# LiHaoxu/SpMV-Research

Measured on AMD Instinct MI355X. Metric: GFLOP/s (2*nnz/t, fp64 SpMV y=A*x); achieved HBM GB/s and % of peak in 'roofline', higher is better.
Workload: dtype f64; 1 GPU; nlpkkt240 (synthetic twin); format=MI355X_SELLD_64_16384_d_v7, rows=27993600, cols=27993600, nnz=765374392, parallelism=single GPU

## Files before the change

spmv-research_amd/csrc/build_sell.hip:

```cpp
#include "handle.hpp"

namespace spmv {

static std::vector<int>
sigma_sort(const int * rp, long m, long sigma)
{
	std::vector<int> row_of_sorted(std::max<long>(m, 1));
	const long num_windows = (m + sigma - 1) / sigma;
	#pragma omp parallel for num_threads(spmv::host_threads()) schedule(dynamic, 4)
	for (long w = 0; w < num_windows; w++)
	{
		long s = w * sigma, e = std::min(m, s + sigma);
		int maxlen = 0;
		for (long i = s; i < e; i++)
			maxlen = std::max(maxlen, rp[i + 1] - rp[i]);
		std::vector<long> cnt((size_t) maxlen + 2, 0);
		for (long i = s; i < e; i++)
			cnt[maxlen - (rp[i + 1] - rp[i]) + 1]++;
		for (int b = 0; b <= maxlen; b++)
			cnt[b + 1] += cnt[b];
		for (long i = s; i < e; i++)
			row_of_sorted[s + cnt[maxlen - (rp[i + 1] - rp[i])]++] = (int) i;
	}
	return row_of_sorted;
// ... 64 lines not shown
					val[p] = va[js + k];
				}
				else
				{
					col[p] = pad_col;
					val[p] = 0.0;
				}
			}
		}
	}
	A->sell_slices = num_slices;
	A->sell_nnz_ext = nnz_ext;
	A->cfg.map = xcd_map_balanced(slice_ptr.data(), num_slices, slices_per_tile,
			resolve_remap(A->remap, (num_slices + slices_per_tile - 1) / slices_per_tile));
	if (dev_alloc(&A->d_slice_ptr, (size_t) num_slices + 1))
		return 1;
	HIP_TRY(hipMemcpy(A->d_slice_ptr, slice_ptr.data(), ((size_t) num_slices + 1) * sizeof(int64_t), hipMemcpyHostToDevice));
	if (upload_ints(col.data(), (size_t) nnz_ext, &A->d_col))
		return 1;
	if (upload_values(A, val.data(), (size_t) nnz_ext, &A->d_val))
		return 1;
	if (upload_ints(row_of_sorted.data(), (size_t) m, &A->d_row_of_sorted))
		return 1;
	A->mem_footprint = (double) (num_slices + 1) * sizeof(int64_t) + (double) nnz_ext * (A->vbytes + 4) + (double) m * 4;
	return 0;
}

static unsigned long long
sell5_exceptions(const int * rp, const int * ci, const int * rows, long maxlen, int r, bool & hard)
{
	unsigned long long mask = 0;
	hard = false;
	const int * cr = ci + rp[rows[r]];
	for (int l = 0; l < 64; l++)
	{
		const int * cl = ci + rp[rows[l]];
		const int off = cl[0] - cr[0];
		for (long k = 1; k < maxlen; k++)
		{
			const int d = cl[k] - cr[k] - off;
			if (d != 0)
				mask |= 1ull << l;
			if (d < -128 || d > 127)
				hard = true;
		}
	}
	return mask;
}

static void
sell_delta_map(spmv_mi355x_matrix * A, const int64_t * val_ptr)
{
	const long num_slices = A->sell_slices;
	const long spt = sell_slices_per_tile() / A->sell_split;
	A->cfg.map = xcd_map_balanced(val_ptr, num_slices, spt, resolve_remap(A->remap, (num_slices + spt - 1) / spt));
	A->mem_footprint = (double) (num_slices + 1) * 16 + (double) A->sell_val_words * A->vbytes + (double) A->sell_idx_bytes + (double) A->m * 4;
}

static void
sell_delta_install(spmv_mi355x_matrix * A, const SellDeltaArrays & r)
{
	A->d_row_of_sorted = r.row_of_sorted;
	A->d_sell_desc = r.desc;
	A->d_sell_idx = r.idx;
	A->d_val = r.val;
	std::copy(r.mode_counts, r.mode_counts + 4, A->sell_mode_slices);
	A->sell_v7_slices = r.v7_slices;
	A->sell_slices = (long) r.val_ptr.size() - 1;
	A->sell_nnz_ext = r.nnz_ext;
	A->sell_val_words = r.val_words;
	A->sell_idx_bytes = r.idx_bytes;
	sell_delta_map(A, r.val_ptr.data());
}

static void
sell_delta_names(spmv_mi355x_matrix * A, const spmv_mi355x_opts & o)
{
	const char * pf = A->f32 ? "f" : "d";
	const char * v7 = A->sell_v7_slices ? "_v7" : "";
	if (A->sell_split > 1)
		snprintf(A->format_name, sizeof(A->format_name), "MI355X_SELLD_%d_%ld_w%d_%s%s", A->sell_c, A->sell_sigma, A->sell_split, pf, v7);
	else
		snprintf(A->format_name, sizeof(A->format_name), "MI355X_SELLD_%d_%ld_%s%s", A->sell_c, A->sell_sigma, pf, v7);
	snprintf(A->kernel_name, sizeof(A->kernel_name), "sell_delta_kernel");
	if (A->sell_v7_slices && o.nontemporal == 0)
		A->cfg.nt = A->mem_footprint > 192.0 * 1024 * 1024 ? 1 : 0;
}

static int
build_sell_delta(spmv_mi355x_matrix * A, int sell_values, const int * rp, const int * ci, const double * va)
{
	const long m = A->m;
	constexpr int C = SELL_DELTA_C;
	const long sigma = A->sell_sigma;
	const long num_slices = (m + C - 1) / C;
	if (A->convert_on_device)
	{
		SellDeltaArrays r;
		if (sell_delta_convert_device(A->f32, m, A->n, A->nnz, sigma, sell_values, rp, ci, va, r))
			return 1;
		sell_delta_install(A, r);
		return 0;
	}
	const std::vector<int> row_of_sorted = sigma_sort(rp, m, sigma);
	std::vector<int64_t> val_ptr((size_t) num_slices + 1, 0), idx_ptr((size_t) num_slices + 1, 0);
	std::vector<unsigned char> mode((size_t) std::max<long>(num_slices, 1), 4);
	#pragma omp parallel for num_threads(spmv::host_threads()) schedule(dynamic, 64)
	for (long sl = 0; sl < num_slices; sl++)
	{
		long width = 0;
		const long i_e = std::min(m, (sl + 1) * C);
		for (long i = sl * C; i < i_e; i++)
		{
			int o = row_of_sorted[i];
			width = std::max<long>(width, rp[o + 1] - rp[o]);
		}
		const long maxlen = width;
		width = (width + 3) / 4 * 4;
		long maxdelta = 0;
		bool equal_len = (sl + 1) * C <= m && A->n >= C && maxlen > 0;
		for (long i = sl * C; i < i_e && equal_len; i++)
			equal_len = (rp[row_of_sorted[i] + 1] - rp[row_of_sorted[i]]) == maxlen;
		bool rowoff = equal_len;
		bool affine = (sl + 1) * C <= m && A->n >= C && maxlen == 0;
		if (rowoff)
		{
			const int o0 = row_of_sorted[sl * C];
			affine = true;
			for (long i = sl * C; i < i_e && rowoff; i++)
			{
				const int o = row_of_sorted[i];
				const int off = ci[rp[o]] - ci[rp[o0]];
				if (off != (int) (i - sl * C))
					affine = false;
				for (long k = 1; k < maxlen && rowoff; k++)
					rowoff = ci[rp[o] + k] - ci[rp[o0] + k] == off;
			}
			if (!rowoff)
				affine = false;
		}
		for (long k = 0; k < width; k++)
		{
			int lo = 0x7fffffff, hi = -1;
			for (long i = sl * C; i < i_e; i++)
			{
				int o = row_of_sorted[i];
				if (k < rp[o + 1] - rp[o])
				{
					int c = ci[rp[o] + k];
					lo = std::min(lo, c);
					hi = std::max(hi, c);
				}
			}
			if (hi >= 0)
				maxdelta = std::max<long>(maxdelta, (long) hi - lo);
		}
		int ref = -1, nex = 0;
		if (equal_len && !rowoff && !(sell_modes_off() & 4))
			for (int r = 0; r < 4 && ref < 0; r++)
			{
				bool hard;
				const int e = __builtin_popcountll(sell5_exceptions(rp, ci, row_of_sorted.data() + sl * C, maxlen, r, hard));
				if (sell5_accepts(e, hard))
				{
					ref = r;
					nex = e;
				}
// ... 474 lines not shown
```

spmv-research_amd/csrc/kernels_sell.hip:

```cpp

#include <type_traits>

#include "sell_delta_read.hpp"

namespace spmv {

constexpr int SELL_BLOCK = 256;
constexpr int SELL_WAVES = SELL_BLOCK / WAVE;

template <typename T, int C, bool NT>
__global__ __launch_bounds__(SELL_BLOCK) void
sell_kernel(const int64_t * __restrict__ slice_ptr, const int * __restrict__ col, const T * __restrict__ val,
		const int * __restrict__ row_of_sorted, const T * __restrict__ x, T * __restrict__ y,
		int m, int num_slices, int beta, XcdMap map)
{
	unsigned tile = xcd_tile(blockIdx.x, map);
	if (tile == NO_TILE)
		return;
	const int lane = threadIdx.x % WAVE;
	const int slice = tile * SELL_WAVES + threadIdx.x / WAVE;
	if (slice >= num_slices)
		return;
	const int64_t p_s = slice_ptr[slice];
	const int64_t p_e = slice_ptr[slice + 1];
// ... 493 lines not shown
}

template <typename T, int S, bool NT, bool V7>
__global__ __launch_bounds__(SELL_BLOCK) void
sell_delta_split_kernel(const int64_t * __restrict__ desc, const unsigned char * __restrict__ idx, const T * __restrict__ val,
		const int * __restrict__ row_of_sorted, const T * __restrict__ x, T * __restrict__ y,
		int m, int num_slices, int beta, XcdMap map)
{
	constexpr int SPB = SELL_WAVES / S;
	__shared__ T s_part[SELL_WAVES][WAVE];
	unsigned tile = xcd_tile(blockIdx.x, map);
	if (tile == NO_TILE)
		return;
	const int lane = threadIdx.x % WAVE;
	const int wave = threadIdx.x / WAVE;
	const int w = __builtin_amdgcn_readfirstlane(wave % S);
	const int slice = __builtin_amdgcn_readfirstlane((int) (tile * SPB + wave / S));
	T s = 0;
	if (slice < num_slices)
		s = sell_delta_one<T, NT, V7>(desc, slice, idx, val, lane, x, w, S);
	s_part[wave][lane] = s;
	__syncthreads();
	if (w == 0 && slice < num_slices)
	{
		T t = s_part[wave][lane];
		#pragma unroll
		for (int u = 1; u < S; u++)
			t += s_part[wave + u][lane];
		const long sorted_row = (long) slice * WAVE + lane;
		if (sorted_row < m)
		{
			T * yp = y + row_of_sorted[sorted_row];
			*yp = beta ? *yp + t : t;
		}
	}
}

template <typename T, bool V7>
static int
sell_delta_launch(int S, const int64_t * desc, const unsigned char * idx, const void * val, const int * row_of_sorted, const void * x, void * y,
		int m, int num_slices, const LaunchCfg & cfg, hipStream_t stream, long * grid_out)
{
	unsigned grid = xcd_grid(cfg.map);
	if (grid_out)
		*grid_out = grid;
	if (grid == 0)
		return 0;
	#define SELLD_LAUNCH(K) hipLaunchKernelGGL(K, dim3(grid), dim3(SELL_BLOCK), 0, stream, desc, idx, (const T *) val, \
			row_of_sorted, (const T *) x, (T *) y, m, num_slices, cfg.beta, cfg.map)
	if (S == 1)
	{
		if (cfg.nt) SELLD_LAUNCH((sell_delta_kernel<T, true, V7>));
		else        SELLD_LAUNCH((sell_delta_kernel<T, false, V7>));
	}
	else if (S == 2)
	{
		if (cfg.nt) SELLD_LAUNCH((sell_delta_split_kernel<T, 2, true, V7>));
		else        SELLD_LAUNCH((sell_delta_split_kernel<T, 2, false, V7>));
	}
	else if (S == 4)
	{
		if (cfg.nt) SELLD_LAUNCH((sell_delta_split_kernel<T, 4, true, V7>));
		else        SELLD_LAUNCH((sell_delta_split_kernel<T, 4, false, V7>));
	}
	else
	{
		set_error("sell_delta: waves per slice must be 1, 2 or 4 (got %d)", S);
		return 1;
	}
	#undef SELLD_LAUNCH
	HIP_TRY(hipGetLastError());
	return 0;
}

int
launch_sell_delta(bool f32, int waves_per_slice, bool v7, const int64_t * desc, const unsigned char * idx, const void * val, const int * row_of_sorted,
		const void * x, void * y, int m, int num_slices, const LaunchCfg & cfg, hipStream_t stream, long * grid_out)
{
	if (f32 && v7)
	{
		set_error("sell_delta: 7-byte values are fp64 only");
		return 1;
	}
	return f32 ? sell_delta_launch<float, false>(waves_per_slice, desc, idx, val, row_of_sorted, x, y, m, num_slices, cfg, stream, grid_out)
	     : v7  ? sell_delta_launch<double, true>(waves_per_slice, desc, idx, val, row_of_sorted, x, y, m, num_slices, cfg, stream, grid_out)
	           : sell_delta_launch<double, false>(waves_per_slice, desc, idx, val, row_of_sorted, x, y, m, num_slices, cfg, stream, grid_out);
}

template <typename T, int C>
static int
sell_launch_c(const int64_t * slice_ptr, const int * col, const void * val, const int * row_of_sorted, const void * x, void * y,
		int m, int num_slices, const LaunchCfg & cfg, hipStream_t stream, long * grid_out)
{
	unsigned grid = xcd_grid(cfg.map);
	if (grid_out)
		*grid_out = grid;
	if (grid == 0)
		return 0;
	if (cfg.nt)
		hipLaunchKernelGGL((sell_kernel<T, C, true>), dim3(grid), dim3(SELL_BLOCK), 0, stream, slice_ptr, col, (const T *) val,
				row_of_sorted, (const T *) x, (T *) y, m, num_slices, cfg.beta, cfg.map);
	else
		hipLaunchKernelGGL((sell_kernel<T, C, false>), dim3(grid), dim3(SELL_BLOCK), 0, stream, slice_ptr, col, (const T *) val,
				row_of_sorted, (const T *) x, (T *) y, m, num_slices, cfg.beta, cfg.map);
	HIP_TRY(hipGetLastError());
	return 0;
}

template <typename T>
static int
sell_dispatch(int C, const int64_t * slice_ptr, const int * col, const void * val, const int * row_of_sorted, const void * x, void * y,
		int m, int num_slices, const LaunchCfg & cfg, hipStream_t stream, long * grid_out)
{
	if (C == SELL_WIDE_C)
	{
		const unsigned grid = xcd_grid(cfg.map);
		if (grid_out)
			*grid_out = grid;
		if (grid == 0)
			return 0;
		if (cfg.nt)
			hipLaunchKernelGGL((sell_wide_kernel<T, true>), dim3(grid), dim3(SELL_WIDE_C), 0, stream, slice_ptr, col, (const T *) val, row_of_sorted,
					(const T *) x, (T *) y, m, num_slices, cfg.beta, cfg.map);
		else
			hipLaunchKernelGGL((sell_wide_kernel<T, false>), dim3(grid), dim3(SELL_WIDE_C), 0, stream, slice_ptr, col, (const T *) val, row_of_sorted,
					(const T *) x, (T *) y, m, num_slices, cfg.beta, cfg.map);
		HIP_TRY(hipGetLastError());
		return 0;
	}
	switch (C)
	{
		case 16: return sell_launch_c<T, 16>(slice_ptr, col, val, row_of_sorted, x, y, m, num_slices, cfg, stream, grid_out);
		case 32: return sell_launch_c<T, 32>(slice_ptr, col, val, row_of_sorted, x, y, m, num_slices, cfg, stream, grid_out);
		case 64: return sell_launch_c<T, 64>(slice_ptr, col, val, row_of_sorted, x, y, m, num_slices, cfg, stream, grid_out);
	}
	set_error("sell: C must be 16, 32, 64 or 256 (got %d)", C);
	return 1;
}

int
launch_sell(bool f32, int C, const int64_t * slice_ptr, const int * col, const void * val, const int * row_of_sorted,
		const void * x, void * y, int m, int num_slices, const LaunchCfg & cfg, hipStream_t stream, long * grid_out)
{
	return f32 ? sell_dispatch<float>(C, slice_ptr, col, val, row_of_sorted, x, y, m, num_slices, cfg, stream, grid_out)
	           : sell_dispatch<double>(C, slice_ptr, col, val, row_of_sorted, x, y, m, num_slices, cfg, stream, grid_out);
}

}
```

spmv-research_amd/csrc/launch.hpp:

```cpp
#pragma once

#include <vector>

#include "common.hpp"
#include "sell_delta_layout.hpp"

namespace spmv {

struct LaunchCfg {
	XcdMap map;
	int nt;
	int beta;
	int unit;
	double unit_value;
	int kahan;
};

inline long csr_scalar_rows_per_tile() { return 256; }
inline long csr_vector_rows_per_tile(int lanes_per_row, int rows_per_group = 1) { return 256L / lanes_per_row * rows_per_group; }
inline long csr_stream_rows_per_tile(int rows_per_wave) { return 4L * rows_per_wave; }
inline long sell_slices_per_tile() { return 4; }
inline long coo_waves_per_tile() { return 4; }

int launch_csr_scalar(bool f32, const int * row_ptr, const int * col, const void * val, const void * x, void * y,
		int m, const LaunchCfg & cfg, hipStream_t stream, long * grid_out);
int launch_csr_vector(bool f32, int lanes_per_row, int rows_per_group, const int * row_ptr, const int * col, const void * val,
		const void * x, void * y, int m, const LaunchCfg & cfg, hipStream_t stream, long * grid_out);

int csr_stream_cap();
int launch_csr_stream(bool f32, int rows_per_wave, const int * row_ptr, const int * col, const void * val, const void * x, void * y,
		int m, const LaunchCfg & cfg, hipStream_t stream, long * grid_out);

int csr_stream_t_cap(int rows_per_wave);
int launch_csr_stream_t(bool f32, int rows_per_wave, const int * row_ptr, const int * col, const void * val, const void * x, void * y,
		int m, const LaunchCfg & cfg, hipStream_t stream, long * grid_out);

int csr_stream_d_cap(int rows_per_wave);
long csr_stream_d_rows_per_tile(int rows_per_wave);
int launch_csr_stream_d(bool f32, int rows_per_wave, const int * row_ptr, const int * col, const void * val, const void * x, void * y,
		int m, const LaunchCfg & cfg, hipStream_t stream, long * grid_out);
constexpr int STREAM_SLACK = 512;

int csr_window_lds_budget();
int launch_csr_window(bool f32, int lanes_per_row, const int * row_ptr, const void * col, int col16, const void * val, const void * x, void * y,
		const int * blk_row, const int * blk_lo, const int * blk_w, int lds_bytes, const LaunchCfg & cfg, hipStream_t stream,
		long * grid_out);

int merge_tile_items(bool f32, int items_per_thread);
int launch_merge_search(const int * row_ptr, int m, int nnz, int tile_items, int num_tiles, int * coords ,
		hipStream_t stream);
int launch_merge(bool f32, int items_per_thread, const int * row_ptr, const int * col, const void * val, const void * x, void * y,
		int m, int nnz, int num_tiles, const int * coords, int * carry_row, void * carry_val,
		const LaunchCfg & cfg, hipStream_t stream, long * grid_out);

int launch_sell(bool f32, int C, const int64_t * slice_ptr, const int * col, const void * val, const int * row_of_sorted,
		const void * x, void * y, int m, int num_slices, const LaunchCfg & cfg, hipStream_t stream, long * grid_out);

int launch_sell_delta(bool f32, int waves_per_slice, bool v7, const int64_t * desc, const unsigned char * idx, const void * val, const int * row_of_sorted,
		const void * x, void * y, int m, int num_slices, const LaunchCfg & cfg, hipStream_t stream, long * grid_out);

int launch_sell_delta_spmm(bool f32, int waves_per_slice, bool v7, const int64_t * desc, const unsigned char * idx, const void * val,
		const int * row_of_sorted, int k, const void * X, long ldx, void * Y, long ldy, int m, int num_slices, const LaunchCfg & cfg,
		hipStream_t stream, long * grid_out);
int launch_spmm_column_gather(bool f32, const void * X, long ldx, void * x, long n, hipStream_t stream);
int launch_spmm_column_scatter(bool f32, const void * y, void * Y, long ldy, long m, int beta, hipStream_t stream);

int sell_window_lds_budget();
int launch_sell_window(bool f32, int waves_per_slice, int slices_per_group, const int * grp, const int64_t * sdesc, const unsigned short * idx,
		const void * val, const int * row_of_sorted, const void * x, void * y, int m, int lds_window_bytes, const LaunchCfg & cfg,
		hipStream_t stream, long * grid_out);

int launch_sell_window_sym(bool f32, int waves_per_slice, int slices_per_group, const int * grp, const int64_t * sdesc, const unsigned short * idx,
		const void * val, const int * row_of_sorted, const void * x, void * y, int m, int lds_window_bytes, const LaunchCfg & cfg,
		hipStream_t stream, long * grid_out);

inline int
sell_modes_off()
{
	const char * e = getenv("SPMV_MI355X_SELL_MODES_OFF");
	return e ? atoi(e) & 7 : 0;
}

inline int
sell_values_env(int opt)
{
	const char * e = getenv("SPMV_MI355X_SELL_VALUES");
	return e ? atoi(e) : opt;
}

__host__ __device__ inline long
sellw_val_pos(long k, long r, bool f32)
{
	return f32 ? (k / 4) * 256 + r * 4 + (k & 3) : (k / 2) * 128 + r * 2 + (k & 1);
}

struct SellDeltaArrays {
	int * row_of_sorted = nullptr;
	int64_t * desc = nullptr;
	unsigned char * idx = nullptr;
	void * val = nullptr;
	std::vector<int64_t> val_ptr;
	long mode_counts[4] = {0, 0, 0, 0};
	int64_t nnz_ext = 0;
	int64_t idx_bytes = 0;
	int64_t val_words = 0;
	long v7_slices = 0;
};

int sell_delta_convert_device(bool f32, long m, long n_cols, long nnz, long sigma, int sell_values, const int * rp_host, const int * ci_host,
		const double * va_host, SellDeltaArrays & out);

int sell_delta_convert_resident(bool f32, long m, long n_cols, long nnz, long sigma, int sell_values, const int * rp, const int * ci,
		const double * va, SellDeltaArrays & out);
int blocked_entries_convert_device(bool f32, bool uniform, long m, long nnz, const int * rp_host, const int * ci_host, const double * va_host, long NR, int WGS, long CH,
		const std::vector<int> & range_row, const std::vector<int> & range_long, const std::vector<int> & long_row, const std::vector<int> & chunk_ptr,
		const std::vector<int> & chunk_row, const std::vector<int> & wg_rows, long SPAN, long BATCH, int slot_bits, int SPARE, long ghost_batches,
		std::vector<int> & batch_ptr, unsigned ** d_ent_out, void ** d_val_out, int ** d_batch_base_out);
int sell_plain_convert_device(bool f32, long m, long nnz, int C, int TPR, long sigma, const int * rp_host, const int * ci_host, const double * va_host,
		int64_t ** d_slice_ptr_out, int ** d_col_out, void ** d_val_out, int ** d_row_of_sorted_out, std::vector<int64_t> & slice_ptr_host);
int sell_window_convert_device(bool f32, long m, long nnz, int NS, bool sym, long lds_budget_bytes, const int * rp_host, const int * ci_host,
		const double * va_host, int ** d_grp_out, int ** d_row_of_sorted_out, int64_t ** d_desc_out, unsigned short ** d_idx_out, void ** d_val_out,
		std::vector<int64_t> & desc_host, int * max_w_out);

int coo_wave_items(int items_per_lane);
int launch_coo(bool f32, int items_per_lane, const int * rowind, const int * col, const void * val, const void * x, void * y,
		int m, long nnz, int num_waves, int * carry_row, void * carry_val,
		const LaunchCfg & cfg, hipStream_t stream, long * grid_out);

int coo_blocked_rows_cap(bool f32);
int coo_blocked_wgs_per_range();
int coo_blocked_chunk_rows();
int coo_blocked_batch_entries(bool unit);
int coo_blocked_spare_slots();
int coo_blocked_slot_bits();
int coo_blocked_max_long_rows();
int launch_coo_blocked(bool f32, const int * wg_rows, const int * range_row, const int * chunk_ptr, const int * chunk_row, const int * batch_ptr, const int * batch_base,
		const int * range_long,
		const int * long_row, int num_long, const unsigned * ent, const void * val, const void * x, void * y, void * carry, int num_ranges,
		int chunk_rows, int lds_bytes, const LaunchCfg & cfg, hipStream_t stream, long * grid_out);

int launch_expand_rows(const int * row_ptr, int m, int * rowind, hipStream_t stream);

}
```

spmv-research_amd/csrc/sell_delta_read.hpp:

```cpp
#pragma once

#include "launch.hpp"

namespace spmv {

typedef int sell_int4 __attribute__((ext_vector_type(4)));
typedef unsigned sell_uint2 __attribute__((ext_vector_type(2)));

template <typename T, bool NT>
__device__ __forceinline__ void
sell_group_values(const T * __restrict__ vp, T (&v)[4])
{
	typedef T T2 __attribute__((ext_vector_type(2)));
	const T2 w0 = ld_stream<NT>(reinterpret_cast<const T2 *>(vp));
	const T2 w1 = ld_stream<NT>(reinterpret_cast<const T2 *>(vp + 2 * WAVE));
	v[0] = w0.x;
	v[1] = w0.y;
	v[2] = w1.x;
	v[3] = w1.y;
}

template <typename T, bool NT, int NSTEPS>
__device__ __forceinline__ void
sell_tail_values(const T * __restrict__ vp, int lane, T (&v)[3])
{
	typedef T T2 __attribute__((ext_vector_type(2)));
	v[1] = v[2] = T(0);
	if (NSTEPS == 1)
		v[0] = ld_stream<NT>(vp - lane);
	else
	{
		const T2 w0 = ld_stream<NT>(reinterpret_cast<const T2 *>(vp));
		v[0] = w0.x;
		v[1] = w0.y;
		if (NSTEPS == 3)
			v[2] = ld_stream<NT>(vp + 2 * WAVE - lane);
	}
}

typedef unsigned sell_uint4 __attribute__((ext_vector_type(4)));
typedef unsigned sell_uint3 __attribute__((ext_vector_type(3), aligned(4)));

__device__ __forceinline__ double
sell_v7_value(unsigned h, unsigned k, unsigned lo)
{
	return __builtin_bit_cast(double, (unsigned long long) sell_v7_decode_hi(h, k) << 32 | lo);
}

template <typename T, bool NT, bool V7>
struct SellVals {
	const T * vp;
	int lane;
	unsigned k;
	__device__ __forceinline__ void group(int g, T (&v)[4]) const
	{
		if constexpr (!V7)
			sell_group_values<T, NT>(vp + (size_t) g * 4 * WAVE, v);
		else
		{
			static_assert(sizeof(T) == 8, "7-byte values are fp64 only");
			const unsigned char * b = reinterpret_cast<const unsigned char *>(vp) + (size_t) g * (8 * SELL_V7_GROUP_WORDS);
			const sell_uint4 lo = ld_stream<NT>(reinterpret_cast<const sell_uint4 *>(b));
			const sell_uint3 * hp = reinterpret_cast<const sell_uint3 *>(b + 1024 - 4 * lane);
			sell_uint3 hi;
			if constexpr (NT)
				hi = __builtin_nontemporal_load(hp);
			else
				hi = *hp;
			v[0] = sell_v7_value(hi.x, k, lo.x);
			v[1] = sell_v7_value(__builtin_amdgcn_alignbit(hi.y, hi.x, 24), k, lo.y);
			v[2] = sell_v7_value(__builtin_amdgcn_alignbit(hi.z, hi.y, 16), k, lo.z);
			v[3] = sell_v7_value(hi.z >> 8, k, lo.w);
		}
	}
	__device__ __forceinline__ const T * tail(int g) const { return vp + (size_t) g * (V7 ? SELL_V7_GROUP_WORDS : 4 * WAVE); }
};

template <int MODE>
struct SellDeltaIdx {
	sell_int4 base;
	sell_uint2 d;
};

template <int MODE, bool NT>
__device__ __forceinline__ void
sell_delta_load_idx(SellDeltaIdx<MODE> & q, const unsigned char * __restrict__ gp , int lane)
{
	q.base = *reinterpret_cast<const sell_int4 *>(gp);
	if constexpr (MODE == 1)
		q.d.x = ld_stream<NT>(reinterpret_cast<const unsigned *>(gp + 16) + lane);
	else
		q.d = ld_stream<NT>(reinterpret_cast<const sell_uint2 *>(gp + 16) + lane);
}

template <int MODE>
__device__ __forceinline__ void
sell_delta_cols(const SellDeltaIdx<MODE> & q, int (&c)[4])
{
	if constexpr (MODE == 1)
	{
		c[0] = q.base.x + (int) (q.d.x & 255u);
		c[1] = q.base.y + (int) ((q.d.x >> 8) & 255u);
		c[2] = q.base.z + (int) ((q.d.x >> 16) & 255u);
		c[3] = q.base.w + (int) (q.d.x >> 24);
	}
	else
	{
		c[0] = q.base.x + (int) (q.d.x & 0xffffu);
		c[1] = q.base.y + (int) (q.d.x >> 16);
		c[2] = q.base.z + (int) (q.d.y & 0xffffu);
		c[3] = q.base.w + (int) (q.d.y >> 16);
	}
}

struct SellDeltaIdx5 {
	sell_int4 base;
	unsigned d;
	sell_int4 corr;
};

template <bool NT, bool SCALAR>
__device__ __forceinline__ void
sell_delta_load_idx5(SellDeltaIdx5 & q, const unsigned char * __restrict__ gp , int rank)
{
	q.base = *reinterpret_cast<const sell_int4 *>(gp);
	if constexpr (SCALAR)
		q.corr = *reinterpret_cast<const sell_int4 *>(gp + 16);
	else
		q.d = ld_stream<NT>(reinterpret_cast<const unsigned *>(gp + 16) + rank);
}

template <bool SCALAR>
__device__ __forceinline__ void
sell_delta_cols5(const SellDeltaIdx5 & q, bool ex, int lane, int off, const int (&xl)[4], int (&c)[4])
{
	int d;
	if constexpr (SCALAR)
	{
		d = lane == xl[0] ? q.corr.x : 0;
		d = lane == xl[1] ? q.corr.y : d;
		d = lane == xl[2] ? q.corr.z : d;
		d = lane == xl[3] ? q.corr.w : d;
	}
	else
		d = ex ? (int) q.d : 0;
	c[0] = q.base.x + off + ((d << 24) >> 24);
	c[1] = q.base.y + off + ((d << 16) >> 24);
	c[2] = q.base.z + off + ((d << 8) >> 24);
	c[3] = q.base.w + off + (d >> 24);
}

template <int MODE, bool NT>
__device__ __forceinline__ void
sell_group_cols(const unsigned char * __restrict__ gp , int lane, int off, int (&c)[4])
{
	static_assert(MODE >= 0 && MODE <= 4, "mode 5 has its own reader (sell_delta_load_idx5, sell_delta_cols5)");
	if constexpr (MODE == 0 || MODE == 3)
	{
		const sell_int4 base = *reinterpret_cast<const sell_int4 *>(gp);
		c[0] = base.x + off;
// ... 46 lines not shown
```

spmv-research_amd/csrc/spmv_mi355x.hip:

```cpp

#include "handle.hpp"

namespace spmv {

static thread_local char g_err[1024] = "";

void
set_error(const char * fmt, ...)
{
	va_list ap;
	va_start(ap, fmt);
	vsnprintf(g_err, sizeof(g_err), fmt, ap);
	va_end(ap);
}

void
init_handle(spmv_mi355x_matrix * A, int format, int precision, int device, const spmv_mi355x_opts & o, long m, long n, long nnz)
{
	A->format = format;
	A->precision = precision;
	A->f32 = (precision == SPMV_MI355X_F32);
	A->vbytes = A->f32 ? 4 : 8;
	A->device = device;
	A->placement_level = (o.placement == 1 || o.placement == 3 || o.placement == 4) ? o.placement : 0;
// ... 462 lines not shown
		HIP_TRY(hipStreamCreate(&A->stream));
	if (!A->d_y && tune_placement(A))
		return 1;
	return 0;
}

void * spmv_mi355x_x_device(spmv_mi355x_matrix * A) { return ensure_xy(A) ? nullptr : A->d_x; }
void * spmv_mi355x_y_device(spmv_mi355x_matrix * A) { return ensure_xy(A) ? nullptr : A->d_y; }

int
spmv_mi355x_set_always_copy(spmv_mi355x_matrix * A, int on)
{
	A->always_copy = on != 0;
	return 0;
}

int
spmv_mi355x_upload_x(spmv_mi355x_matrix * A, const void * x_host)
{
	if (ensure_xy(A))
		return 1;
	HIP_TRY(hipDeviceSynchronize());
	HIP_TRY(hipMemcpyAsync(A->d_x, x_host, (size_t) A->n * A->vbytes, hipMemcpyHostToDevice, A->stream));
	HIP_TRY(hipStreamSynchronize(A->stream));
	A->cached_x_host = x_host;
	return 0;
}

int
spmv_mi355x_upload_y(spmv_mi355x_matrix * A, const void * y_host)
{
	if (ensure_xy(A))
		return 1;
	HIP_TRY(hipDeviceSynchronize());
	HIP_TRY(hipMemcpyAsync(A->d_y, y_host, (size_t) A->m * A->vbytes, hipMemcpyHostToDevice, A->stream));
	HIP_TRY(hipStreamSynchronize(A->stream));
	return 0;
}

int
spmv_mi355x_download_y(spmv_mi355x_matrix * A, void * y_host)
{
	if (ensure_xy(A))
		return 1;
	HIP_TRY(hipDeviceSynchronize());
	HIP_TRY(hipMemcpyAsync(y_host, A->d_y, (size_t) A->m * A->vbytes, hipMemcpyDeviceToHost, A->stream));
	HIP_TRY(hipStreamSynchronize(A->stream));
	A->y_downloaded = true;
	return 0;
}

int
spmv_mi355x_spmv(spmv_mi355x_matrix * A, const void * x_host, void * y_host)
{
	if (ensure_xy(A))
		return 1;
	if (A->always_copy || A->cached_x_host != x_host)
	{
		if (spmv_mi355x_upload_x(A, x_host))
			return 1;
		A->y_downloaded = false;
	}
	if (spmv_mi355x_spmv_device_async(A, A->d_x, A->d_y, 0, A->stream))
		return 1;
	HIP_TRY(hipStreamSynchronize(A->stream));
	if (A->always_copy || !A->y_downloaded)
		if (spmv_mi355x_download_y(A, y_host))
			return 1;
	return 0;
}

int
spmv_mi355x_stored_array(const spmv_mi355x_matrix * A, const char * name, void ** out, size_t * bytes_out)
{
	if (!A || !name || !out || !bytes_out)
	{
		set_error("stored_array: NULL argument");
		return 1;
	}
	*out = nullptr;
	*bytes_out = 0;
	struct Arr { const char * name; const void * p; size_t bytes; };
	std::vector<Arr> arrs;
	if (A->format == SPMV_MI355X_SELL_C_SIGMA && A->sell_window)
		arrs = {{"val", A->d_val, (size_t) A->sell_nnz_ext * A->vbytes}, {"idx", A->d_sell_idx, (size_t) A->sell_idx_bytes},
		        {"desc", A->d_sell_desc, 2 * ((size_t) A->sell_slices + 1) * 8}, {"row_of_sorted", A->d_row_of_sorted, (size_t) A->m * 4},
		        {"groups", A->d_sellw_grp, (size_t) A->sellw_groups * 16}};
	else if (A->format == SPMV_MI355X_SELL_C_SIGMA && A->sell_delta)
		arrs = {{"val", A->d_val, (size_t) A->sell_val_words * A->vbytes}, {"idx", A->d_sell_idx, (size_t) A->sell_idx_bytes},
		        {"desc", A->d_sell_desc, 2 * ((size_t) A->sell_slices + 1) * 8}, {"row_of_sorted", A->d_row_of_sorted, (size_t) A->m * 4}};
	else if (A->format == SPMV_MI355X_SELL_C_SIGMA)
		arrs = {{"val", A->d_val, (size_t) A->sell_nnz_ext * A->vbytes}, {"col", A->d_col, (size_t) A->sell_nnz_ext * 4},
		        {"slice_ptr", A->d_slice_ptr, ((size_t) A->sell_slices + 1) * 8}, {"row_of_sorted", A->d_row_of_sorted, (size_t) A->m * 4}};
	else if (A->d_coob_ent)
	{
		const size_t NT = (size_t) A->coob_ranges * spmv::coo_blocked_wgs_per_range(), BATCH = (size_t) spmv::coo_blocked_batch_entries(A->cfg.unit != 0);
		const size_t stored = ((size_t) A->coob_batches + 2) * BATCH;
		arrs = {{"entries", A->d_coob_ent, stored * 4}, {"val", A->d_val, A->cfg.unit ? 0 : stored * A->vbytes},
		        {"batch_base", A->d_coob_batch_base, stored / 64 * 4}, {"batch_ptr", A->d_coob_batch_ptr, (NT + 1) * 4},
		        {"chunk_ptr", A->d_coob_chunk_ptr, (NT + 1) * 4}, {"chunk_row", A->d_coob_chunk_row, (size_t) A->coob_chunks * 4},
		        {"wg_rows", A->d_coob_wg_rows, NT * 4}, {"range_row", A->d_coob_range_row, ((size_t) A->coob_ranges + 1) * 4},
		        {"range_long", A->d_coob_range_long, ((size_t) A->coob_ranges + 1) * 4}, {"long_row", A->d_coob_long_row, (size_t) A->coob_num_long * 4}};
	}
	else
	{
		set_error("stored_array: only for the SELL layouts and the column-blocked layout (this handle: %s)", A->format_name);
		return 1;
	}
	for (const Arr & a : arrs)
		if (!strcmp(a.name, name))
		{
			HIP_TRY(hipSetDevice(A->device));
			void * host = malloc(std::max<size_t>(a.bytes, 1));
			if (!host)
			{
				set_error("stored_array: out of host memory (%zu bytes)", a.bytes);
				return 1;
			}
			if (a.bytes && hipMemcpy(host, a.p, a.bytes, hipMemcpyDeviceToHost) != hipSuccess)
			{
				free(host);
				set_error("stored_array: copy failed: %s", hipGetErrorString(hipGetLastError()));
				return 1;
			}
			*out = host;
			*bytes_out = a.bytes;
			return 0;
		}
	set_error("stored_array: %s has no array '%s'", A->format_name, name);
	return 1;
}

int
spmv_mi355x_sell_layout(const spmv_mi355x_matrix * A, long * C_out, long * sigma_out, long * num_slices_out,
		long * nnz_ext_out, int64_t ** slice_ptr_out, int32_t ** col_out, double ** val_out, int32_t ** row_of_sorted_out)
{
	if (A->format != SPMV_MI355X_SELL_C_SIGMA)
	{
		set_error("not a SELL handle");
		return 1;
	}
	if (A->sell_window)
	{
		set_error("sell_layout: not available for the LDS-window layout (16-bit window-relative indices)");
		return 1;
	}
	HIP_TRY(hipSetDevice(A->device));
	if (C_out) *C_out = A->sell_c;
	if (sigma_out) *sigma_out = A->sell_sigma;
	if (num_slices_out) *num_slices_out = A->sell_slices;
	if (nnz_ext_out) *nnz_ext_out = A->sell_nnz_ext;
	std::vector<int64_t> h_desc, plain_ptr;
	std::vector<unsigned char> h_idx;
	if (A->sell_delta)
	{
		h_desc.resize(2 * ((size_t) A->sell_slices + 1));
		HIP_TRY(hipMemcpy(h_desc.data(), A->d_sell_desc, h_desc.size() * sizeof(int64_t), hipMemcpyDeviceToHost));
		h_idx.resize((size_t) std::max<long>(A->sell_idx_bytes, 1));
		HIP_TRY(hipMemcpy(h_idx.data(), A->d_sell_idx, (size_t) A->sell_idx_bytes, hipMemcpyDeviceToHost));
		plain_ptr.assign((size_t) A->sell_slices + 1, 0);
		for (long sl = 0; sl < A->sell_slices; sl++)
		{
			const long width = spmv::sell_slice_width(h_desc[2 * sl + 2] - h_desc[2 * sl], spmv::sell_desc_v7(h_desc[2 * sl + 1]));
			plain_ptr[sl + 1] = plain_ptr[sl] + width * 64;
		}
	}
// ... 134 lines not shown
```

Measured before the change: 1415 GFLOP/s.

## Add producer-wave LDS ring kernel for SELL-delta fp64 SpMV

Adds a new SELL-delta kernel in which a dedicated producer wave streams slice values into a double-buffered LDS ring with global_load_lds DMA, while four consumer waves gather x and run FMAs on values read from LDS. It is enabled automatically for fp64 single-wave slices when the extended value array exceeds 256 MiB, with a persistent grid capped per XCD. The aim is to overlap value streaming with x gathers and keep more bytes in flight toward HBM bandwidth. In exchange it adds block-wide barriers per round, imbalance when the four slices in a tile differ in length, and fewer resident workgroups.

```diff
diff --git a/spmv-research_amd/csrc/build_sell.hip b/spmv-research_amd/csrc/build_sell.hip
--- a/spmv-research_amd/csrc/build_sell.hip
+++ b/spmv-research_amd/csrc/build_sell.hip
@@ -170,7 +170,10 @@
 		snprintf(A->format_name, sizeof(A->format_name), "MI355X_SELLD_%d_%ld_w%d_%s%s", A->sell_c, A->sell_sigma, A->sell_split, pf, v7);
 	else
 		snprintf(A->format_name, sizeof(A->format_name), "MI355X_SELLD_%d_%ld_%s%s", A->sell_c, A->sell_sigma, pf, v7);
-	snprintf(A->kernel_name, sizeof(A->kernel_name), "sell_delta_kernel");
+	A->cfg.ring = sell_ring_wanted(A->f32, A->sell_split, A->sell_nnz_ext) ? 1 : 0;
+	snprintf(A->kernel_name, sizeof(A->kernel_name), A->cfg.ring ? "sell_delta_ring_kernel" : "sell_delta_kernel");
+	if (A->cfg.ring)
+		A->kernel_block = 320;
 	if (A->sell_v7_slices && o.nontemporal == 0)
 		A->cfg.nt = A->mem_footprint > 192.0 * 1024 * 1024 ? 1 : 0;
 }
diff --git a/spmv-research_amd/csrc/kernels_sell.hip b/spmv-research_amd/csrc/kernels_sell.hip
--- a/spmv-research_amd/csrc/kernels_sell.hip
+++ b/spmv-research_amd/csrc/kernels_sell.hip
@@ -599,6 +599,9 @@
 		set_error("sell_delta: 7-byte values are fp64 only");
 		return 1;
 	}
+	if (cfg.ring && !f32 && waves_per_slice == 1)
+		return launch_sell_delta_ring(v7, desc, idx, (const double *) val, row_of_sorted, (const double *) x, (double *) y, m, num_slices, cfg, stream,
+				grid_out);
 	return f32 ? sell_delta_launch<float, false>(waves_per_slice, desc, idx, val, row_of_sorted, x, y, m, num_slices, cfg, stream, grid_out)
 	     : v7  ? sell_delta_launch<double, true>(waves_per_slice, desc, idx, val, row_of_sorted, x, y, m, num_slices, cfg, stream, grid_out)
 	           : sell_delta_launch<double, false>(waves_per_slice, desc, idx, val, row_of_sorted, x, y, m, num_slices, cfg, stream, grid_out);
diff --git a/spmv-research_amd/csrc/kernels_sell_ring.hip b/spmv-research_amd/csrc/kernels_sell_ring.hip
--- /dev/null
+++ b/spmv-research_amd/csrc/kernels_sell_ring.hip
@@ -0,0 +1,339 @@
+
+#include "sell_delta_read.hpp"
+
+namespace spmv {
+
+constexpr int RING_NC = 4;
+constexpr int RING_D = 2;
+constexpr int RING_BLOCK = (RING_NC + 1) * WAVE;
+constexpr int RING_WG_PER_XCD = 32 * 2;
+constexpr int RING_LDS_BYTES = RING_NC * RING_D * SELL_RING_SLOT_BYTES;
+static_assert(RING_LDS_BYTES <= 65536, "the LDS-DMA destination base must stay below 64 KiB");
+
+struct RingSlice {
+	int64_t v_off, i_word;
+	int width, full;
+	bool v7;
+};
+
+template <bool V7>
+__device__ __forceinline__ RingSlice
+ring_slice_info(const int64_t * __restrict__ desc, int slice, int num_slices)
+{
+	RingSlice r{0, 0, 0, 0, false};
+	if (slice < num_slices)
+	{
+		r.v_off = desc[2 * slice];
+		r.i_word = desc[2 * slice + 1];
+		r.v7 = V7 && sell_desc_v7(r.i_word);
+		r.width = (int) sell_slice_width(desc[2 * slice + 2] - r.v_off, r.v7);
+		r.full = r.width / 4;
+	}
+	return r;
+}
+
+__device__ __forceinline__ int ring_trips(int full) { return (full + SELL_RING_SLOT_GROUPS - 1) / SELL_RING_SLOT_GROUPS; }
+
+template <bool V7>
+__device__ __forceinline__ int
+ring_tile_rounds(const int64_t * __restrict__ desc, unsigned tile, int num_slices)
+{
+	int R = 0;
+	#pragma unroll
+	for (int c = 0; c < RING_NC; c++)
+	{
+		const int t = ring_trips(ring_slice_info<V7>(desc, (int) (tile * RING_NC + c), num_slices).full);
+		R = t > R ? t : R;
+	}
+	return R;
+}
+
+template <typename F>
+__device__ __forceinline__ void
+ring_walk(const XcdMap & map, unsigned blocks, F && f)
+{
+	for (unsigned vb = blockIdx.x; vb < blocks; vb += gridDim.x)
+	{
+		const unsigned tile = xcd_tile(vb, map);
+		if (tile != NO_TILE)
+			f(tile);
+	}
+}
+
+__device__ __forceinline__ void
+ring_barrier()
+{
+	asm volatile("s_waitcnt lgkmcnt(0)" ::: "memory");
+	__builtin_amdgcn_s_barrier();
+	asm volatile("" ::: "memory");
+}
+
+__device__ __forceinline__ void
+ring_pin(double & v)
+{
+	asm volatile("" : "+v"(v));
+}
+
+template <int MODE, bool NT, bool V7, bool SC5>
+__device__ __forceinline__ double
+ring_slice(const RingSlice & si, const unsigned char * __restrict__ ip, int off, unsigned long long mask, const double * __restrict__ val,
+		const void * safe, int lane, const double * __restrict__ x, const unsigned char * slots, int & rnd)
+{
+	typedef double double2_t __attribute__((ext_vector_type(2)));
+	const int full = si.full, rem = si.width - 4 * full, trips = ring_trips(full), groups = (si.width + 3) / 4;
+	const Sell5Lane<SC5> l5(mask, lane);
+	const size_t GB = MODE == 5 ? sell_group_bytes(5, (unsigned) __popcll(mask)) : sell_group_bytes(MODE);
+	auto cols = [&](int g, int (&c)[4]) {
+		const unsigned char * gp = ip + (size_t) g * GB;
+		if constexpr (MODE == 5)
+		{
+			SellDeltaIdx5 q;
+			sell_delta_load_idx5<NT, SC5>(q, gp, l5.rank);
+			sell_delta_cols5<SC5>(q, l5.ex, lane, off, l5.xl, c);
+		}
+		else
+			sell_group_cols<MODE, NT>(gp, lane, off, c);
+	};
+	const double * tp = val + si.v_off + (size_t) full * (si.v7 ? SELL_V7_GROUP_WORDS : 4 * WAVE);
+	const double2_t * pa = rem >= 2 ? reinterpret_cast<const double2_t *>(tp + 2 * lane) : reinterpret_cast<const double2_t *>(safe);
+	const double * pb = rem == 1 ? tp + lane : rem == 3 ? tp + 2 * WAVE + lane : reinterpret_cast<const double *>(safe);
+	const double2_t ta = ld_stream<NT>(pa);
+	const double tb = ld_stream<NT>(pb);
+	const double tv0 = rem == 1 ? tb : ta.x, tv1 = ta.y, tv2 = tb;
+	int ct[4];
+	cols(groups - 1, ct);
+	const double tx0 = x[ct[0]], tx1 = x[ct[1]], tx2 = x[ct[2]];
+
+	const SellRingVals<V7> rv{lane, V7 ? (unsigned) (sell_v7_e0(si.i_word) - 1) << 20 : 0u};
+	double s = 0;
+	auto gather = [&](int q, double (&xx)[4][4]) {
+		#pragma unroll
+		for (int u = 0; u < 4; u++)
+		{
+			int g = 4 * q + u;
+			g = g < full ? g : full - 1;
+			int c[4];
+			cols(g, c);
+			#pragma unroll
+			for (int t = 0; t < 4; t++)
+				xx[u][t] = x[c[t]];
+		}
+	};
+	auto consume = [&](int q, const double (&xx)[4][4]) {
+		ring_barrier();
+		const unsigned char * slot = slots + (rnd % RING_D) * SELL_RING_SLOT_BYTES;
+		rnd++;
+		double v[4][4];
+		#pragma unroll
+		for (int u = 0; u < 4; u++)
+			rv.group(slot, u, v[u]);
+		#pragma unroll
+		for (int u = 0; u < 4; u++)
+			if (4 * q + u < full)
+			{
+				#pragma unroll
+				for (int t = 0; t < 4; t++)
+					s = fma(v[u][t], xx[u][t], s);
+			}
+	};
+	if (trips > 0)
+	{
+		double xa[4][4];
+		gather(0, xa);
+		for (int q = 0; q + 1 < trips; q++)
+		{
+			double xb[4][4];
+			gather(q + 1, xb);
+			consume(q, xa);
+			#pragma unroll
+			for (int u = 0; u < 4; u++)
+				#pragma unroll
+				for (int t = 0; t < 4; t++)
+				{
+					ring_pin(xb[u][t]);
+					xa[u][t] = xb[u][t];
+				}
+		}
+		consume(trips - 1, xa);
+	}
+	if (rem > 0) s = fma(tv0, tx0, s);
+	if (rem > 1) s = fma(tv1, tx1, s);
+	if (rem > 2) s = fma(tv2, tx2, s);
+	return s;
+}
+
+template <bool NT, bool V7, bool SV7>
+__device__ __forceinline__ double
+ring_slice_modes(const RingSlice & si, const unsigned char * __restrict__ idx, const double * __restrict__ val, const void * safe, int lane,
+		const double * __restrict__ x, const unsigned char * slots, int & rnd)
+{
+	const unsigned char * ip = idx + sell_desc_idx(si.i_word);
+	const int mode = sell_desc_mode(si.i_word);
+	if (mode == 0)
+		return ring_slice<0, NT, SV7, false>(si, ip, lane, 0ull, val, safe, lane, x, slots, rnd);
+	if (mode == 1)
+		return ring_slice<1, NT, SV7, false>(si, ip, lane, 0ull, val, safe, lane, x, slots, rnd);
+	if (mode == 2)
+		return ring_slice<2, NT, SV7, false>(si, ip, lane, 0ull, val, safe, lane, x, slots, rnd);
+	if (mode == 4)
+		return ring_slice<4, NT, SV7, false>(si, ip, lane, 0ull, val, safe, lane, x, slots, rnd);
+	const int off = ld_stream<NT>(reinterpret_cast<const int *>(ip) + lane);
+	if (mode == 3)
+		return ring_slice<3, NT, SV7, false>(si, ip + sell_header_bytes(3), off, 0ull, val, safe, lane, x, slots, rnd);
+	const unsigned long long mask = *reinterpret_cast<const unsigned long long *>(ip + 4 * WAVE);
+	if (__popcll(mask) <= 4)
+		return ring_slice<5, NT, SV7, true>(si, ip + sell_header_bytes(5), off, mask, val, safe, lane, x, slots, rnd);
+	return ring_slice<5, NT, SV7, false>(si, ip + sell_header_bytes(5), off, mask, val, safe, lane, x, slots, rnd);
+}
+
+typedef __attribute__((address_space(1))) const void ring_gvoid;
+typedef __attribute__((address_space(3))) void ring_lvoid;
+
+template <typename T, bool NT, bool V7>
+__global__ __launch_bounds__(RING_BLOCK) void
+sell_delta_ring_kernel(const int64_t * __restrict__ desc, const unsigned char * __restrict__ idx, const T * __restrict__ val,
+		const int * __restrict__ row_of_sorted, const T * __restrict__ x, T * __restrict__ y,
+		int m, int num_slices, int beta, XcdMap map, unsigned blocks)
+{
+	static_assert(sizeof(T) == 8, "the ring kernel is fp64 only");
+	__shared__ __attribute__((aligned(16))) unsigned char ring[RING_LDS_BYTES];
+	const int lane = threadIdx.x % WAVE;
+	const int wave = __builtin_amdgcn_readfirstlane((int) (threadIdx.x / WAVE));
+	int rnd = 0;
+	if (wave == RING_NC)
+	{
+		ring_walk(map, blocks, [&](unsigned tile) {
+			RingSlice si[RING_NC];
+			int R = 0;
+			#pragma unroll
+			for (int c = 0; c < RING_NC; c++)
+			{
+				si[c] = ring_slice_info<V7>(desc, (int) (tile * RING_NC + c), num_slices);
+				const int t = ring_trips(si[c].full);
+				R = t > R ? t : R;
+			}
+			for (int q = 0; q < R; q++)
+			{
+				unsigned char * base = ring + (rnd % RING_D) * SELL_RING_SLOT_BYTES;
+				#pragma unroll
+				for (int c = 0; c < RING_NC; c++)
+				{
+					const int n = si[c].full - SELL_RING_SLOT_GROUPS * q;
+					const size_t gb = si[c].v7 ? 8 * SELL_V7_GROUP_WORDS : SELL_RING_GROUP_BYTES;
+					const unsigned char * src = reinterpret_cast<const unsigned char *>(val + si[c].v_off) + (size_t) SELL_RING_SLOT_GROUPS * q * gb;
+					unsigned char * dst = base + c * RING_D * SELL_RING_SLOT_BYTES;
+					#pragma unroll
+					for (int u = 0; u < SELL_RING_SLOT_GROUPS; u++)
+						if (u < n)
+						{
+							const unsigned char * g = src + u * gb;
+							unsigned char * l = dst + u * SELL_RING_GROUP_BYTES;
+							__builtin_amdgcn_global_load_lds((ring_gvoid *) (g + 16 * lane), (ring_lvoid *) l, 16, 0, NT ? 2 : 0);
+							if (si[c].v7)
+								__builtin_amdgcn_global_load_lds((ring_gvoid *) (g + 1024 + 12 * lane), (ring_lvoid *) (l + 1024), 12, 0, NT ? 2 : 0);
+							else
+								__builtin_amdgcn_global_load_lds((ring_gvoid *) (g + 1024 + 16 * lane), (ring_lvoid *) (l + 1024), 16, 0, NT ? 2 : 0);
+						}
+				}
+				asm volatile("s_waitcnt vmcnt(0)" ::: "memory");
+				ring_barrier();
+				rnd++;
+			}
+		});
+		return;
+	}
+	const unsigned char * slots = ring + wave * RING_D * SELL_RING_SLOT_BYTES;
+	ring_walk(map, blocks, [&](unsigned tile) {
+		const int R = ring_tile_rounds<V7>(desc, tile, num_slices);
+		const int slice = (int) (tile * RING_NC + wave);
+		const RingSlice si = ring_slice_info<V7>(desc, slice, num_slices);
+		const int r0 = rnd;
+		if (si.width > 0)
+		{
+			const long sorted_row = (long) slice * WAVE + lane;
+			const int yrow = row_of_sorted[sorted_row < m ? sorted_row : m - 1];
+			const T s = (V7 && si.v7) ? ring_slice_modes<NT, V7, true>(si, idx, val, desc, lane, x, slots, rnd)
+			                          : ring_slice_modes<NT, V7, false>(si, idx, val, desc, lane, x, slots, rnd);
+			if (sorted_row < m)
+			{
+				T * yp = y + yrow;
+				*yp = beta ? *yp + s : s;
+			}
+		}
+		else if (slice < num_slices)
+		{
+			const long sorted_row = (long) slice * WAVE + lane;
+			if (sorted_row < m && !beta)
+				y[row_of_sorted[sorted_row]] = T(0);
+		}
+		for (int q = rnd - r0; q < R; q++)
+		{
+			ring_barrier();
+			rnd++;
+		}
+	});
+}
+
+template <bool V7>
+__global__ void
+sell_ring_rounds_kernel(const int64_t * __restrict__ desc, int num_slices, XcdMap map, unsigned blocks, int * __restrict__ out)
+{
+	int B = 0;
+	ring_walk(map, blocks, [&](unsigned tile) { B += ring_tile_rounds<V7>(desc, tile, num_slices); });
+	if (threadIdx.x == 0)
+		out[blockIdx.x] = B;
+}
+
+unsigned
+sell_ring_grid(const XcdMap & map)
+{
+	const unsigned blocks = xcd_grid(map), fit = NUM_XCD * RING_WG_PER_XCD;
+	return blocks < fit ? blocks : fit;
+}
+
+int
+launch_sell_delta_ring(bool v7, const int64_t * desc, const unsigned char * idx, const double * val, const int * row_of_sorted,
+		const double * x, double * y, int m, int num_slices, const LaunchCfg & cfg, hipStream_t stream, long * grid_out)
+{
+	const unsigned blocks = xcd_grid(cfg.map), grid = sell_ring_grid(cfg.map);
+	if (grid_out)
+		*grid_out = grid;
+	if (grid == 0)
+		return 0;
+	#define RING_LAUNCH(NT, V7) hipLaunchKernelGGL((sell_delta_ring_kernel<double, NT, V7>), dim3(grid), dim3(RING_BLOCK), 0, stream, desc, idx, val, \
+			row_of_sorted, x, y, m, num_slices, cfg.beta, cfg.map, blocks)
+	if (v7)
+	{
+		if (cfg.nt) RING_LAUNCH(true, true);
+		else        RING_LAUNCH(false, true);
+	}
+	else
+	{
+		if (cfg.nt) RING_LAUNCH(true, false);
+		else        RING_LAUNCH(false, false);
+	}
+	#undef RING_LAUNCH
+	HIP_TRY(hipGetLastError());
+	return 0;
+}
+
+int
+sell_ring_rounds(bool v7, const int64_t * desc, int num_slices, const LaunchCfg & cfg, std::vector<int> & out)
+{
+	const unsigned blocks = xcd_grid(cfg.map), grid = sell_ring_grid(cfg.map);
+	out.assign(grid, 0);
+	if (grid == 0)
+		return 0;
+	int * d = nullptr;
+	HIP_TRY(hipMalloc((void **) &d, grid * sizeof(int)));
+	if (v7)
+		hipLaunchKernelGGL(sell_ring_rounds_kernel<true>, dim3(grid), dim3(WAVE), 0, 0, desc, num_slices, cfg.map, blocks, d);
+	else
+		hipLaunchKernelGGL(sell_ring_rounds_kernel<false>, dim3(grid), dim3(WAVE), 0, 0, desc, num_slices, cfg.map, blocks, d);
+	const hipError_t e = hipMemcpy(out.data(), d, grid * sizeof(int), hipMemcpyDeviceToHost);
+	(void) hipFree(d);
+	HIP_TRY(e);
+	return 0;
+}
+
+}
diff --git a/spmv-research_amd/csrc/launch.hpp b/spmv-research_amd/csrc/launch.hpp
--- a/spmv-research_amd/csrc/launch.hpp
+++ b/spmv-research_amd/csrc/launch.hpp
@@ -14,6 +14,7 @@
 	int unit;
 	double unit_value;
 	int kahan;
+	int ring;
 };
 
 inline long csr_scalar_rows_per_tile() { return 256; }
@@ -59,6 +60,10 @@
 int launch_sell_delta(bool f32, int waves_per_slice, bool v7, const int64_t * desc, const unsigned char * idx, const void * val, const int * row_of_sorted,
 		const void * x, void * y, int m, int num_slices, const LaunchCfg & cfg, hipStream_t stream, long * grid_out);
 
+int launch_sell_delta_ring(bool v7, const int64_t * desc, const unsigned char * idx, const double * val, const int * row_of_sorted,
+		const double * x, double * y, int m, int num_slices, const LaunchCfg & cfg, hipStream_t stream, long * grid_out);
+int sell_ring_rounds(bool v7, const int64_t * desc, int num_slices, const LaunchCfg & cfg, std::vector<int> & out);
+
 int launch_sell_delta_spmm(bool f32, int waves_per_slice, bool v7, const int64_t * desc, const unsigned char * idx, const void * val,
 		const int * row_of_sorted, int k, const void * X, long ldx, void * Y, long ldy, int m, int num_slices, const LaunchCfg & cfg,
 		hipStream_t stream, long * grid_out);
@@ -86,6 +91,17 @@
 {
 	const char * e = getenv("SPMV_MI355X_SELL_VALUES");
 	return e ? atoi(e) : opt;
+}
+
+constexpr bool SELL_RING_AUTO = true;
+inline bool
+sell_ring_wanted(bool f32, int waves_per_slice, int64_t nnz_ext)
+{
+	const char * e = getenv("SPMV_MI355X_SELL_RING");
+	const int v = e ? atoi(e) : 0;
+	if (f32 || waves_per_slice != 1 || v == 2)
+		return false;
+	return v == 1 || (SELL_RING_AUTO && (double) nnz_ext * 8 > 256.0 * 1024 * 1024);
 }
 
 __host__ __device__ inline long
diff --git a/spmv-research_amd/csrc/sell_delta_read.hpp b/spmv-research_amd/csrc/sell_delta_read.hpp
--- a/spmv-research_amd/csrc/sell_delta_read.hpp
+++ b/spmv-research_amd/csrc/sell_delta_read.hpp
@@ -76,6 +76,39 @@
 	__device__ __forceinline__ const T * tail(int g) const { return vp + (size_t) g * (V7 ? SELL_V7_GROUP_WORDS : 4 * WAVE); }
 };
 
+constexpr int SELL_RING_SLOT_GROUPS = 4;
+constexpr int SELL_RING_GROUP_BYTES = 2048;
+constexpr int SELL_RING_SLOT_BYTES = SELL_RING_SLOT_GROUPS * SELL_RING_GROUP_BYTES;
+
+template <bool V7>
+struct SellRingVals {
+	int lane;
+	unsigned k;
+	__device__ __forceinline__ void group(const unsigned char * slot, int u, double (&v)[4]) const
+	{
+		const unsigned char * b = slot + u * SELL_RING_GROUP_BYTES;
+		if constexpr (!V7)
+		{
+			typedef double double2_t __attribute__((ext_vector_type(2)));
+			const double2_t w0 = *reinterpret_cast<const double2_t *>(b + 16 * lane);
+			const double2_t w1 = *reinterpret_cast<const double2_t *>(b + 1024 + 16 * lane);
+			v[0] = w0.x;
+			v[1] = w0.y;
+			v[2] = w1.x;
+			v[3] = w1.y;
+		}
+		else
+		{
+			const sell_uint4 lo = *reinterpret_cast<const sell_uint4 *>(b + 16 * lane);
+			const sell_uint3 hi = *reinterpret_cast<const sell_uint3 *>(b + 1024 + 12 * lane);
+			v[0] = sell_v7_value(hi.x, k, lo.x);
+			v[1] = sell_v7_value(__builtin_amdgcn_alignbit(hi.y, hi.x, 24), k, lo.y);
+			v[2] = sell_v7_value(__builtin_amdgcn_alignbit(hi.z, hi.y, 16), k, lo.z);
+			v[3] = sell_v7_value(hi.z >> 8, k, lo.w);
+		}
+	}
+};
+
 template <int MODE>
 struct SellDeltaIdx {
 	sell_int4 base;
diff --git a/spmv-research_amd/csrc/spmv_mi355x.hip b/spmv-research_amd/csrc/spmv_mi355x.hip
--- a/spmv-research_amd/csrc/spmv_mi355x.hip
+++ b/spmv-research_amd/csrc/spmv_mi355x.hip
@@ -568,6 +568,23 @@
 	*bytes_out = 0;
 	struct Arr { const char * name; const void * p; size_t bytes; };
 	std::vector<Arr> arrs;
+	if (A->format == SPMV_MI355X_SELL_C_SIGMA && A->sell_delta && !A->sell_window && A->cfg.ring && !strcmp(name, "ring_rounds"))
+	{
+		HIP_TRY(hipSetDevice(A->device));
+		std::vector<int> rounds;
+		if (spmv::sell_ring_rounds(A->sell_v7_slices > 0, A->d_sell_desc, (int) A->sell_slices, A->cfg, rounds))
+			return 1;
+		void * host = malloc(std::max<size_t>(rounds.size() * sizeof(int), 1));
+		if (!host)
+		{
+			set_error("stored_array: out of host memory");
+			return 1;
+		}
+		memcpy(host, rounds.data(), rounds.size() * sizeof(int));
+		*out = host;
+		*bytes_out = rounds.size() * sizeof(int);
+		return 0;
+	}
 	if (A->format == SPMV_MI355X_SELL_C_SIGMA && A->sell_window)
 		arrs = {{"val", A->d_val, (size_t) A->sell_nnz_ext * A->vbytes}, {"idx", A->d_sell_idx, (size_t) A->sell_idx_bytes},
 		        {"desc", A->d_sell_desc, 2 * ((size_t) A->sell_slices + 1) * 8}, {"row_of_sorted", A->d_row_of_sorted, (size_t) A->m * 4},
```

New measurement: 597.6 GFLOP/s. 0.422x the previous value.
